# fperezgamonal/flownet2-tf

Measured on AMD Instinct MI355X. Metric: forward pairs/sec at 512x384 (FlowNet2), higher is better.
Workload: dtype f16x2 (split fp16 hi+lo operands, 3 fp16 MFMAs per product, fp32 accumulate); 1 GPU; FlowNet2 forward, batch=4 synthetic 512x384 pairs per GPU, seeded synthetic weights; pairs_per_gpu=4, parallelism=dp1 (no collective)

## Files before the change

### flownet2-tf_amd/csrc/conv.hip

```cpp
#include "conv_common.h"
#include <cstdlib>

namespace fn2 {

template <typename T, typename OutT, int TC, int WC, int WP>
__global__ void __launch_bounds__(256) conv_igemm_kernel(const ConvArgs p) {
  constexpr int CH = 16 / (int)sizeof(T);
  constexpr int BC = WC * TC * 16;
  constexpr int BP = WP * 64;
  constexpr int NT = 256;
  static_assert(WC * WP == 4, "4 waves per block");
  constexpr int NPR = BP / 64;
  constexpr int NWR = (BC * 4 + NT - 1) / NT;
  constexpr int WSWZ_BIT = (TC == 4) ? 5 : (TC == 2) ? 4 : 3;
  __shared__ uint4 lds[2][(BC + BP) * 4];

  const int tid = threadIdx.x, lane = tid & 63, wave = tid >> 6;
  const int wc = wave / WP, wp = wave % WP;
  const int cid = tid & 3;

  int pad_y = p.pad, pad_x = p.pad, oy_off = 0, ox_off = 0, osc = 1;
  const T* wgt = reinterpret_cast<const T*>(p.wgt);
  const int phase = blockIdx.z / p.splitk, split = blockIdx.z - phase * p.splitk;
  if (p.deconv) {
// ... 970 lines not shown
  {
    const double A = (double)d->cout_pad * d->kpad * esz, B = (double)d->in.n * d->in.h * d->in.w * d->in.cs * esz;
    const long X = cdiv(M, 64), Y = cdiv(d->cout_pad, 128);
    const char* e = getenv("FN2_WMAJOR");
    const int mode = e ? atoi(e) : 2;
    a.wmajor = mode == 2 ? (A * (double)(X < 8 ? X : 8) + B > A + B * (double)(Y < 8 ? Y : 8)) : mode;
  }
  a.bp64 = wfrag ? 1 : wants_bp64(a, tile, phases, d->wgt_layout) ? 1 : 0;
  if ((a.dbg & 64) && d->wgt_layout == 1 && tile == 128 && !a.bp64) a.bp64 = 2;
  if (wfrag) {
    const char* e_wr = getenv("FN2_WREG_RING");
    const char* e_ring = getenv("FN2_RING_MAX");
    const int mode = e_wr ? atoi(e_wr) : 1;
    const long blocks = (long)cdiv(a.M, 64) * (a.cout_pad / 128) * phases;
    if (tile == 128 && (mode == 2 || (mode == 1 && blocks >= 384 && blocks <= (e_ring ? atoi(e_ring) : 512)))) a.wfrag = 2;
  }
  a.kg = 1;
  if (d->wgt_layout == 1 && tile == 128 && !(a.dbg & 32)) {
    const char* e_kg = getenv("FN2_KG");
    if (!e_kg || atoi(e_kg) != 0) {
      const char* e3 = getenv("FN2_KG3_MAX");
      const char* e2 = getenv("FN2_KG2_MAX");
      const long blocks = (long)cdiv(a.M, 64) * (a.cout_pad / 128) * phases;
      if (blocks <= (e3 ? atoi(e3) : 0)) { a.bp64 = 1; a.kg = 3; }
      else if (blocks <= (e2 ? atoi(e2) : 95)) { a.bp64 = 1; a.kg = 2; }
    }
  }
  if (d->wgt_layout == 1 && tile == 128 && !(a.dbg & 32) && d->in.dtype == FN2_F16X2) {
    const char* e_lo = getenv("FN2_DEEP_MIN");
    const char* e_hi = getenv("FN2_DEEP_MAX");
// ... 2 lines not shown
    if (blocks >= lo && blocks <= hi) { a.bp64 = 3; a.kg = 1; }
  }
  if (d->wgt_layout == 1 && tile == 128 && a.bp64 == 1 && a.kg == 1) {
    const char* e_ring = getenv("FN2_RING_MAX");
    const int ring_max = e_ring ? atoi(e_ring) : 512;
    const long blocks = (long)cdiv(a.M, 64) * (a.cout_pad / 128) * phases;
    if ((a.dbg & 256) || (blocks >= 384 && blocks <= ring_max)) a.bp64 = 2;
    const char* e_rs = getenv("FN2_RING_SPLIT");
    if (e_rs && blocks >= atoi(e_rs) && blocks < 384) a.bp64 = 2;
  }
  *tile_out = tile;
  *phases_out = phases;
  return FN2_OK;
}

static int preferred_split(const ConvArgs& a, int tile, int phases) {
  if (a.merged) return 1;
  const int bp = tile == 128 ? (a.bp64 ? 64 : 128) : (a.bp64 ? 128 : 256);
  const long blocks = (long)cdiv(a.M, bp) * (a.cout_pad / tile) * phases;
  const char* e_min = getenv("FN2_SPLIT_MINBLOCKS");
  if (blocks >= (e_min ? atoi(e_min) : 384)) return 1;
  if (a.bp64 == 3) {
    const char* e_sl = getenv("FN2_DEEP_SLOTS");
    int s = (int)((e_sl ? atoi(e_sl) : 256) / blocks);
    const int maxs = a.ksteps / 16;
    if (s > maxs) s = maxs;
    if (s > 16) s = 16;
    if (s < 2) return 1;
    const int kper = cdiv(a.ksteps, s);
    return cdiv(a.ksteps, kper);
  }
  if (a.kg > 1) {
// ... 101 lines not shown
  if (d->up_src != nullptr && d->kind == 5 && 2 * d->out.c == 32) {
    a.up_src = d->up_src; a.up_w = d->up_w; a.up_bias = d->up_bias; a.up_c0 = d->up_c0;
  }
  if (d->head != nullptr && !conv_name_sink().buf) {
    const fn2_conv_desc* h = reinterpret_cast<const fn2_conv_desc*>(d->head);
    FN2_REQUIRE(d->kind == 1 && is_flow_head(h) && h->head == nullptr && h->up_src == nullptr,
                "conv2d: head rides on a kind-1 transposed conv and is a 3x3 two-output fp32 flow head");
    FN2_REQUIRE(h->in.data == d->in.data && h->in.n == d->in.n && h->in.h == d->in.h && h->in.w == d->in.w &&
                    h->in.cs == d->in.cs && h->in.c0 == d->in.c0 && h->in.dtype == d->in.dtype,
                "conv2d: head and transposed conv must read the same view");
    ConvArgs ha;
    int htile, hphases;
    rc = build_args(h, &ha, &htile, &hphases);
    if (rc) return rc;
    const char* e = getenv("FN2_HEAD_RIDE");
    const bool ride = d->in.dtype == FN2_F16X2 && d->wgt_layout == 2 && tile == 128 && sk > 1 && !(e && atoi(e) == 0);
    if (ride) {
      a.fh_M = ha.M;
      a.fh_w = reinterpret_cast<const float*>(ha.wgt);
      a.fh_w1 = ha.ksteps * 4 * 4;
      a.fh_groups = ha.cin_chunks >> 1;
      a.fh_bias = ha.bias;
      a.fh_out = reinterpret_cast<float*>(ha.out);
      a.fh_out_cs = ha.out_cs; a.fh_out_c0 = ha.out_c0;
      a.fh_scale = ha.out_scale;
    } else {
      rc = fn2_conv2d(h, stream);
      if (rc) return rc;
    }
  }
  if (d->wgt_layout >= 1) {
// ... 220 lines not shown
```

### flownet2-tf_amd/csrc/conv2.hip

```cpp
#include "conv_common.h"

#include <type_traits>
#include <algorithm>
#include <utility>

#ifndef FN2_X2_ORDER
#define FN2_X2_ORDER 0
#endif
#ifndef FN2_CONV_ABLATE
#define FN2_CONV_ABLATE 0
#endif
#ifndef FN2_SETPRIO
#define FN2_SETPRIO 1
#endif

namespace fn2 {

typedef __attribute__((address_space(3))) void* lptr_t;

constexpr unsigned kOobOffset = 0x80000000u;

typedef int v4i_t __attribute__((ext_vector_type(4)));
typedef unsigned u32x4_t __attribute__((ext_vector_type(4)));

// ... 74 lines not shown
  for (int k = 0; k < 4; ++k) {
    const long m = (long)rb * 16 + wave * 4 + k;
    if (m >= total) return;
    h5_ring_pixel(p, m);
  }
}

__device__ __forceinline__ float* h5_t(uint4* a, uint4* b, int half, int w) {
  const int byte = w * 4;
  return byte < half ? reinterpret_cast<float*>(reinterpret_cast<char*>(a) + byte)
                     : reinterpret_cast<float*>(reinterpret_cast<char*>(b) + (byte - half));
}

template <typename T, typename OutT, int WC, int WP, int TCN = 2, int TPN = 2, int STAGES = 2, int KG = 1, bool M16 = false,
          bool WREG = false, bool SLAB = false, bool HEAD5 = false, bool FEED = false>
__global__ void __launch_bounds__(256 * KG + (FEED ? 256 : 0)) conv_igemm2_kernel(const ConvArgs p) {
#if defined(__HIP_DEVICE_COMPILE__)
  constexpr int CH = 16 / (int)sizeof(T);
  constexpr int ESZ = (int)sizeof(T);
  constexpr int BC = WC * TCN * 32, BP = WP * TPN * 32;
  static_assert(WC * WP == 4, "4 waves per block");
  constexpr int NWI = BC / 32;
  constexpr int NPI = BP / 32;
  static_assert(!WREG || (is_x2<T>::value && TCN == 1 && KG == 1 && (STAGES == 2 || STAGES == 3) && !M16),
                "WREG: split fp16, one cout tile per wave, two-stage loop or 3-slot ring");
  constexpr int BOFF = WREG ? 0 : BC;
  constexpr int kWTileBytes = (32 * TPN * (TCN * 32 + 4) + 32 * TPN) * 4;
  constexpr int kPoolHalfRows = (STAGES * BP * 128 / 2 > 2 * kWTileBytes ? STAGES * BP * 128 / 2 : 2 * kWTileBytes) / 128 + 1;
  constexpr int ROWS = WREG ? kPoolHalfRows : BC + BP;
  static_assert(KG == 1 || STAGES == 2, "K groups run the two-stage loop");
  constexpr bool kDeep = STAGES > 3;
  __shared__ uint4 lds0_all[(kDeep ? STAGES : WREG ? 2 : KG) * ROWS * 8];
  __shared__ uint4 lds1_all[(kDeep || WREG) ? 1 : KG * ROWS * 8];
  __shared__ uint4 lds2_own[(STAGES == 3 && !WREG) ? ROWS * 8 : 1];

  if constexpr (HEAD5) {
    if ((int)blockIdx.x >= p.h5_tiles) {
      h5_ring_block(p, (int)blockIdx.x - p.h5_tiles);
      return;
    }
  }
  if constexpr (WREG && SLAB && is_x2<T>::value) {
    if (p.fh_M > 0 && (int)blockIdx.z >= p.fh_z0) {
      if (FEED && threadIdx.x >= 256) return;
      float* part = reinterpret_cast<float*>(lds0_all);
      const long e = (((long)blockIdx.z - p.fh_z0) * gridDim.y + blockIdx.y) * gridDim.x + blockIdx.x;
      const long total = (long)(gridDim.z - p.fh_z0) * gridDim.y * gridDim.x;
      for (long m = e; m < p.fh_M; m += total)
        fh_pixel(reinterpret_cast<const x2_t*>(p.in), p.H, p.W, p.in_cs, p.in_c0, p.fh_groups, p.fh_w, p.fh_w + p.fh_w1,
                 p.fh_bias, p.fh_scale, p.fh_out + (size_t)m * p.fh_out_cs + p.fh_out_c0, m, part);
      return;
    }
  }
  const int tid = threadIdx.x, lane = tid & 63;
  const int wave_all = __builtin_amdgcn_readfirstlane(tid >> 6);
  const int grp = KG > 1 ? wave_all >> 2 : 0;
  static_assert(!FEED || (WREG && STAGES == 3 && KG == 1), "FEED: the WREG ring");
  const bool feeder = FEED && wave_all >= 4;
  const int wave = (KG > 1 || FEED) ? wave_all & 3 : wave_all;
  uint4* const lds0 = lds0_all + grp * (ROWS * 8);
  uint4* const lds1 = WREG ? lds0_all + BP * 8 : kDeep ? lds0_all + ROWS * 8 : lds1_all + grp * (ROWS * 8);
  uint4* const lds2 = WREG ? lds0_all + 2 * BP * 8 : lds2_own;
  uint4* const ep1 = (kDeep || WREG) ? lds0_all + ROWS * 8 : lds1_all;
  const int wc = wave / WP, wp = wave % WP;

  int pad_y = p.pad, pad_x = p.pad, oy_off = 0, ox_off = 0, osc = 1;
  const T* wgt = reinterpret_cast<const T*>(p.wgt);
  const int phase = blockIdx.z / p.splitk, split = blockIdx.z - phase * p.splitk;
  const unsigned wrow_bytes = (unsigned)p.ksteps * 128u;
  if (p.deconv) {
    const int a = phase >> 1, b = phase & 1;
    pad_y = a ? p.ph_pad1 : p.ph_pad0; pad_x = b ? p.ph_pad1 : p.ph_pad0; oy_off = a; ox_off = b; osc = 2;
    wgt += (size_t)phase * p.cout_pad * (wrow_bytes / ESZ);
  }
  const int khi = p.deconv ? p.kh_ph[phase >> 1] : p.KH, kwi = p.deconv ? p.kw_ph[phase & 1] : p.KW;
  const int nst_all = (p.cin_chunks >> 3) * khi * kwi;
// ... 17 lines not shown

  const v4i_t rsrc_w = make_rsrc(wgt, (int)(p.cout_pad * wrow_bytes));
  const v4i_t rsrc_x = make_rsrc(p.in, p.in_bytes);

  const int lrow = lane >> 3, lphys = lane & 7;
  unsigned woff[NWI];
#pragma unroll
  for (int j = 0; j < NWI; ++j) {
    const int row = wave * (BC / 4) + j * 8 + lrow;
    woff[j] = (unsigned)(c0 + row) * wrow_bytes + (unsigned)((lphys ^ ((row >> 1) & 7)) * 16);
  }
  int roff[NPI];
  unsigned vmask[NPI];
#pragma unroll
  for (int j = 0; j < NPI; ++j) {
    const int row = wave * (BP / 4) + j * 8 + lrow;
    const int m = m0 + row;
    bool v = m < p.M;
    const int mm = v ? m : 0;
    int n = mm / (p.OH * p.OW);
    const int rem = mm - n * (p.OH * p.OW);
    int oy = rem / p.OW, ox = rem - oy * p.OW;
    if constexpr (HEAD5) {
      static_assert(BP == 256, "HEAD5: 8 x 32 positions per block");
      const int tx = bx % p.h5_tx, tyn = bx / p.h5_tx;
      n = tyn / p.h5_ty;
      oy = (tyn - n * p.h5_ty) * 4 - 2 + (row >> 5);
      ox = tx * 28 - 2 + (row & 31);
      v = true;
    }
    const int iy0 = oy * p.stride - pad_y, ix0 = ox * p.stride - pad_x;
// ... 14 lines not shown
  int wstage = kt0;

  auto issue_piece = [&](auto piece_c, uint4* lds) {
    constexpr int i = decltype(piece_c)::value;
    if constexpr (i < NWI) {
      if constexpr (!WREG) {
        if (!(FN2_CONV_ABLATE && (p.dbg & 2)))
          dma16(rsrc_w, &lds[(wave * (BC / 4) + i * 8) * 8], woff[i], ((ky * p.KW + kx) * spt + sc) * 128);
      }
    } else {
      constexpr int j = i - NWI;
      const unsigned tbit = (1u << ky) | (1u << (8 + kx));
      const int toff = ((ky * p.W + kx) * p.in_cs + sc * 8 * CH) * ESZ;
      const unsigned voff = ((vmask[j] & tbit) == tbit && wstage < kt1) ? (unsigned)(roff[j] + toff) : kOobOffset;
      if (!(FN2_CONV_ABLATE && (p.dbg & 1)))
        dma16(rsrc_x, &lds[(BOFF + wave * (BP / 4) + j * 8) * 8], voff, 0);
    }
  };
  u32x4_t wfa[WREG ? 4 : 1], wfb[WREG ? 4 : 1], wfc[(WREG && STAGES == 3) ? 4 : 1];
  const unsigned wlane = (unsigned)lane * 16u;
  const int wtile_off = WREG ? ((c0 >> 5) + wc) * (p.ksteps * 4096) : 0;
  auto load_w = [&](u32x4_t (&wf)[WREG ? 4 : 1]) {
    if constexpr (WREG) {
      const int soff = wtile_off + ((ky * p.KW + kx) * spt + sc) * 4096;
      asm volatile("buffer_load_dwordx4 %0, %4, %5, %6 offen\n\t"
                   "buffer_load_dwordx4 %1, %4, %5, %6 offen offset:1024\n\t"
                   "buffer_load_dwordx4 %2, %4, %5, %6 offen offset:2048\n\t"
                   "buffer_load_dwordx4 %3, %4, %5, %6 offen offset:3072"
                   : "=&v"(wf[0]), "=&v"(wf[1]), "=&v"(wf[2]), "=&v"(wf[3])
                   : "v"(wlane), "s"(rsrc_w), "s"(soff) : "memory");
    }
// ... 206 lines not shown
    };
    issue_stage_w(lds0, wfa);
    issue_stage_w(lds1, wfb);
    const int nst3 = (kt1 - kt0 + 2) / 3 * 3;
    for (int s = 0; s < nst3; s += 3) {
      ring_sync_w(wfa); issue_stage_w(lds2, wfc); compute_w(lds0, wfa);
      ring_sync_w(wfb); issue_stage_w(lds0, wfa); compute_w(lds1, wfb);
      ring_sync_w(wfc); issue_stage_w(lds1, wfb); compute_w(lds2, wfc);
    }
    asm volatile("s_waitcnt vmcnt(0)" : "+v"(wfa[0]), "+v"(wfa[1]), "+v"(wfa[2]), "+v"(wfa[3]), "+v"(wfb[0]), "+v"(wfb[1]),
                 "+v"(wfb[2]), "+v"(wfb[3]) :: "memory");
  } else if constexpr (WREG) {
    issue_stage_w(lds0, wfa);
    wait_w(wfa);
    __syncthreads();
    const int nst2 = (kt1 - kt0 + 1) & ~1;
    for (int s = 0; s < nst2; s += 2) {
      issue_stage_w(lds1, wfb);
      compute_w(lds0, wfa);
      wait_w(wfb);
      __syncthreads();
      if (s + 2 < nst2) issue_stage_w(lds0, wfa);
      compute_w(lds1, wfb);
      wait_w(wfa);
      __syncthreads();
    }
  } else if constexpr (STAGES == 2) {
    issue_stage(lds0);
    asm volatile("s_waitcnt vmcnt(0)" ::: "memory");
    __syncthreads();
    const int nst2 = ((kt1 - (kt0 - grp) + KG - 1) / KG + 1) & ~1;
// ... 32 lines not shown
      else asm volatile("s_waitcnt vmcnt(8)\n\ts_barrier" ::: "memory");
    };
    issue_stage(lds0);
    issue_stage(lds1);
    const int nst3 = (kt1 - kt0 + 2) / 3 * 3;
    for (int s = 0; s < nst3; s += 3) {
      ring_sync(); issue_stage(lds2); compute(lds0);
      ring_sync(); issue_stage(lds0); compute(lds1);
      ring_sync(); issue_stage(lds1); compute(lds2);
    }
    asm volatile("s_waitcnt vmcnt(0)" ::: "memory");
  }

  if constexpr (KG > 1) {
    constexpr int NA4 = TCN * TPN * 4;
    static_assert((KG - 1) * 4 * NA4 * 64 <= KG * ROWS * 8, "reduction scratch must fit the stage buffers");
    float4* red = reinterpret_cast<float4*>(lds0_all);
    auto acc4 = [&](int idx) -> float4 {
      if constexpr (M16) {
        const f32x4 v = acc16[idx / (TPN * 2)][idx % (TPN * 2)];
        return make_float4(v[0], v[1], v[2], v[3]);
      } else {
        const int t = idx >> 2, q = idx & 3;
        return make_float4(acc[t / TPN][t % TPN][4 * q], acc[t / TPN][t % TPN][4 * q + 1], acc[t / TPN][t % TPN][4 * q + 2],
                           acc[t / TPN][t % TPN][4 * q + 3]);
      }
    };
    if (grp > 0) {
#pragma unroll
      for (int idx = 0; idx < NA4; ++idx) red[(((grp - 1) * 4 + wave) * NA4 + idx) * 64 + lane] = acc4(idx);
    }
    __syncthreads();
    if (grp > 0) return;
#pragma unroll
    for (int g = 0; g < KG - 1; ++g)
#pragma unroll
      for (int idx = 0; idx < NA4; ++idx) {
        const float4 v = red[((g * 4 + wave) * NA4 + idx) * 64 + lane];
        if constexpr (M16) {
          f32x4& d = acc16[idx / (TPN * 2)][idx % (TPN * 2)];
          d[0] += v.x; d[1] += v.y; d[2] += v.z; d[3] += v.w;
        } else {
          const int t = idx >> 2, q = idx & 3;
          acc[t / TPN][t % TPN][4 * q] += v.x; acc[t / TPN][t % TPN][4 * q + 1] += v.y;
          acc[t / TPN][t % TPN][4 * q + 2] += v.z; acc[t / TPN][t % TPN][4 * q + 3] += v.w;
        }
      }
  }

  if constexpr (HEAD5) {
    if (p.dbg & 2) return;
    constexpr int TS = 52;
    static_assert(256 * TS * 4 <= 2 * ROWS * 128, "T fits the stage buffers");
// ... 66 lines not shown
          v[j] = x;
        }
        if (p.vec_ok && co + 3 < p.Cout) store_vec<OutT, 4>(po + co, v);
        else
#pragma unroll
          for (int j = 0; j < 4; ++j)
            if (co + j < p.Cout) store_elem<OutT>(po + co + j, v[j]);
      }
    }
    return;
  }

  OutT* out = reinterpret_cast<OutT*>(p.out);
  constexpr int WCOLS = TCN * 32, RS = WCOLS + 4, WROWS = 32 * TPN;
  constexpr int WTW = WROWS * RS + WROWS;
  constexpr bool kLdsT = (KG > 1 ? 4 : 2) * WTW * 4 <= KG * ROWS * 128;
  if constexpr (FEED && !kLdsT) { if (feeder) return; }
  float* const tl = reinterpret_cast<float*>(KG > 1 ? ep1 : (wave < 2 ? lds0_all : ep1)) + (KG > 1 ? wave : (wave & 1)) * WTW;
  constexpr int CPR = WCOLS / 4, RPI = 64 / CPR;
  static_assert(!SLAB || WREG, "SLAB is a specialisation of the WREG instantiations");
  if ((SLAB || !WREG) && p.splitk > 1) {
    float* slab = p.ws + (size_t)split * p.N * p.out_H * p.out_W * p.ws_cs;
    if constexpr (kLdsT) {
      if constexpr (STAGES >= 3) __syncthreads();
      if constexpr (FEED) { if (feeder) return; }
      int* rowoff = reinterpret_cast<int*>(tl + WROWS * RS);
#pragma unroll
      for (int tp = 0; tp < TPN; ++tp) {
        const int m = m0 + wp * TPN * 32 + tp * 32 + fr;
        const int mm = m < p.M ? m : 0;
        const int n = mm / (p.OH * p.OW);
        const int rem = mm - n * (p.OH * p.OW);
        const int oy = rem / p.OW, ox = rem - oy * p.OW;
// ... 810 lines not shown
  const char* e_m16 = getenv("FN2_M16_MIN");
  const bool m16 = is_x2<T>::value && !(a.dbg & 512) &&
                   ((a.dbg & 1024) || (e_m16 && tile == 128 && a.bp64 == 1 && a.kg == 1 && a.splitk == 1 &&
                                       blocks64 >= atoi(e_m16)));
#define FN2_LAUNCH2(GX, GY, THREADS, ...)                                                              \
  do {                                                                                                 \
    dim3 grid(GX, GY, z);                                                                              \
    if (conv_name_sink().buf)                                                                          \
      snprintf(conv_name_sink().buf, conv_name_sink().cap, "conv_igemm2_kernel<%s, %s, %s, %s>", type_name<T>(), \
               type_name<OutT>(), #__VA_ARGS__, m16 ? "true" : "false");                              \
    else if (m16) hipLaunchKernelGGL((conv_igemm2_kernel<T, OutT, __VA_ARGS__, is_x2<T>::value>), grid, dim3(THREADS), 0, s, a); \
    else hipLaunchKernelGGL((conv_igemm2_kernel<T, OutT, __VA_ARGS__, false>), grid, dim3(THREADS), 0, s, a);            \
  } while (0)
  if (a.wfrag) {
    if constexpr (is_x2<T>::value) {
      if (tile == 64) {
        dim3 grid(cdiv(a.M, 128), a.cout_pad / 64, z);
        if (conv_name_sink().buf)
          snprintf(conv_name_sink().buf, conv_name_sink().cap, "conv_igemm2_kernel<%s, %s, 2, 2, 1, 2, 2, 1, false, true, %s>",
                   type_name<T>(), type_name<OutT>(), a.splitk > 1 ? "true" : "false");
        else if (a.splitk > 1)
          hipLaunchKernelGGL((conv_igemm2_kernel<T, OutT, 2, 2, 1, 2, 2, 1, false, true, true>), grid, dim3(256), 0, s, a);
        else
          hipLaunchKernelGGL((conv_igemm2_kernel<T, OutT, 2, 2, 1, 2, 2, 1, false, true, false>), grid, dim3(256), 0, s, a);
      } else {
        dim3 grid(cdiv(a.M, 64), a.cout_pad / 128, z);
        const bool slab = a.splitk > 1;
        ConvArgs ah = a;
        if (a.fh_M > 0 && slab && !conv_name_sink().buf) {
          const char* e = getenv("FN2_FH_BLOCKS");
          const long per_z = (long)grid.x * grid.y;
          const long want = std::min<long>(a.fh_M, e ? atoi(e) : 1024);
          ah.fh_z0 = z;
          grid.z = z + (unsigned)std::max<long>(1, (want + per_z - 1) / per_z);
        } else {
          ah.fh_M = 0;
        }
        const ConvArgs& a = ah;
        const char* e_feed = getenv("FN2_WREG_FEED");
        const int feed = e_feed ? atoi(e_feed) : 1;
        if (conv_name_sink().buf)
          snprintf(conv_name_sink().buf, conv_name_sink().cap, "conv_igemm2_kernel<%s, %s, 4, 1, 1, 2, %d, 1, false, true, %s%s>",
                   type_name<T>(), type_name<OutT>(), a.wfrag == 2 ? 3 : 2, slab ? "true" : "false",
                   (a.wfrag == 2 && (slab ? feed >= 2 : feed >= 1)) ? ", false, true" : "");
        else if (a.wfrag == 2 && slab && feed >= 2)
          hipLaunchKernelGGL((conv_igemm2_kernel<T, OutT, 4, 1, 1, 2, 3, 1, false, true, true, false, true>), grid, dim3(512), 0, s, a);
        else if (a.wfrag == 2 && slab)
          hipLaunchKernelGGL((conv_igemm2_kernel<T, OutT, 4, 1, 1, 2, 3, 1, false, true, true>), grid, dim3(256), 0, s, a);
        else if (a.wfrag == 2 && feed >= 1)
          hipLaunchKernelGGL((conv_igemm2_kernel<T, OutT, 4, 1, 1, 2, 3, 1, false, true, false, false, true>), grid, dim3(512), 0, s, a);
        else if (a.wfrag == 2)
          hipLaunchKernelGGL((conv_igemm2_kernel<T, OutT, 4, 1, 1, 2, 3, 1, false, true, false>), grid, dim3(256), 0, s, a);
        else if (slab)
          hipLaunchKernelGGL((conv_igemm2_kernel<T, OutT, 4, 1, 1, 2, 2, 1, false, true, true>), grid, dim3(256), 0, s, a);
        else
          hipLaunchKernelGGL((conv_igemm2_kernel<T, OutT, 4, 1, 1, 2, 2, 1, false, true, false>), grid, dim3(256), 0, s, a);
// ... 64 lines not shown
```

### flownet2-tf_amd/csrc/conv_common.h

```cpp
#pragma once
#include "fn2_common.h"

namespace fn2 {

struct ConvArgs {
  const void* in;
  const void* wgt;
  const float* bias;
  void* out;
  int N, H, W, in_cs, in_c0;
  int cin_chunks;
  int KH, KW, stride, pad;
  int OH, OW;
  int M;
  int out_H, out_W, out_cs, out_c0, Cout;
  int ksteps;
  int cout_pad;
  int act;
  int deconv;
  int ph_pad0, ph_pad1;
  int kh_ph[2], kw_ph[2];
  int merged;
  int wmajor;
  int bp64;
// ... 1 lines not shown
  int kg;
  int h5_tx, h5_ty, h5_ring;
  int h5_tiles, h5_groups;
  const float* h5_wc;
  const float* h5_bc;
  int h5_rows;
  int fh_M, fh_z0;
  const float* fh_w;
  int fh_w1, fh_groups;
  const float* fh_bias;
  float* fh_out;
  int fh_out_cs, fh_out_c0;
  float fh_scale;
  const float* up_src; const float* up_w; const float* up_bias; int up_c0;
  int wfrag;
  int accum;
  int vec_ok;
  int splitk;
  int kper;
  float* ws;
  int ws_cs;
  float out_scale;
  int in_bytes;
  const void* mask_y;
  int mask_c0, mask_c1;
  int dbg;
};

__device__ __forceinline__ void fh_pixel(const x2_t* __restrict__ in, int H, int W, int in_cs, int in_c0, int groups,
                                         const float* __restrict__ wf0, const float* __restrict__ wf1,
// ... 93 lines not shown
```

### flownet2-tf_amd/src/_hip.py

```python
import ctypes as C
import os

import numpy as np
import torch

_HERE = os.path.dirname(os.path.abspath(__file__))
LIB_PATH = os.path.join(os.path.dirname(_HERE), "lib", "libflownet2_hip.so")

FN2_F32, FN2_BF16, FN2_F16, FN2_F16X2 = 0, 1, 2, 3
ACT_NONE, ACT_LEAKY = 0, 1
OK = 0
ERR_INVALID_ARGUMENT, ERR_UNSUPPORTED, ERR_HIP = -1, -2, -3


class Fn2Tensor(C.Structure):
    _fields_ = [("data", C.c_void_p), ("dtype", C.c_int32), ("n", C.c_int32), ("h", C.c_int32),
                ("w", C.c_int32), ("c", C.c_int32), ("cs", C.c_int32), ("c0", C.c_int32)]


class Fn2ConvPlan(C.Structure):
    _fields_ = [("layout", C.c_int32), ("cout_tile", C.c_int32), ("kstep_elems", C.c_int32),
                ("wgt_dtype", C.c_int32)]


class Fn2ConvDesc(C.Structure):
    _fields_ = [("inp", Fn2Tensor), ("out", Fn2Tensor), ("wgt", C.c_void_p), ("bias", C.c_void_p),
                ("kind", C.c_int32), ("kh", C.c_int32), ("kw", C.c_int32), ("stride", C.c_int32),
                ("pad", C.c_int32), ("act", C.c_int32), ("cin_pad", C.c_int32), ("cout_pad", C.c_int32),
                ("kpad", C.c_int32), ("wgt_layout", C.c_int32), ("accumulate", C.c_int32), ("out_scale", C.c_float), ("workspace", C.c_void_p), ("workspace_bytes", C.c_int64),
                ("act_grad_y", C.c_void_p), ("act_grad_c0", C.c_int32), ("act_grad_c1", C.c_int32),
                ("up_src", C.c_void_p), ("up_w", C.c_void_p), ("up_bias", C.c_void_p), ("up_c0", C.c_int32),
                ("head", C.c_void_p), ("raw_partials", C.c_int32)]


class Fn2BwdwDesc(C.Structure):
    _fields_ = [("x", Fn2Tensor), ("dy", Fn2Tensor), ("dw", C.c_void_p), ("kind", C.c_int32), ("kh", C.c_int32),
                ("kw", C.c_int32), ("stride", C.c_int32), ("pad", C.c_int32), ("cin_pad", C.c_int32),
                ("cout_pad", C.c_int32), ("kpad", C.c_int32), ("wgt_layout", C.c_int32), ("db", C.c_void_p)]


_i, _p, _f = C.c_int, C.c_void_p, C.c_float
_ip = C.POINTER(C.c_int)
_tp = C.POINTER(Fn2Tensor)

PROTOTYPES = {
    "fn2_last_error": (C.c_char_p, []),
    "fn2_version": (_i, []),
# ... 150 lines not shown
```

### flownet2-tf_amd/src/engine.py

```python
import ctypes as C
import math
import os

import numpy as np
import torch

from . import _hip, netdefs, weights as W

_DT = {"f32": torch.float32, "bf16": torch.bfloat16, "f16": torch.float16, "f16x2": torch.float32}
_CODE = {"f32": _hip.FN2_F32, "bf16": _hip.FN2_BF16, "f16": _hip.FN2_F16, "f16x2": _hip.FN2_F16X2}
_TILE_ARGS = {128: "2, 2, 2, 2", 64: "1, 4, 2, 2", 32: "1, 4, 1, 2"}


def conv2_kernel_args(tile, m, cout_pad, phases, x2=True):
    dbg = int(os.environ.get("FN2_CONV_DBG", "0"))
    blocks64 = -(-m // 64) * (cout_pad // 128) * phases if tile == 128 else 0
    big = "FN2_M16_MIN" in os.environ and blocks64 >= max(int(os.environ["FN2_M16_MIN"]), 513)
    m16 = "true" if (x2 and not dbg & 512 and (dbg & 1024 or big)) else "false"
    full = dbg & 32
    if tile < 128:
        base = {64: "1, 4, 2, 2, 2, 1", 32: "1, 4, 1, 2, 2, 1"}[tile] if full else {64: "1, 4, 2, 1, 2, 1", 32: "1, 4, 1, 1, 2, 1"}[tile]
        return f"{base}, {m16}"
    blocks = -(-m // 64) * (cout_pad // 128) * phases
    if not full and int(os.environ.get("FN2_KG", "1")):
# ... 15 lines not shown


class BatchTooLarge(ValueError):

    def __init__(self, name, batch, nbytes, limit):
        self.fit = max(1, int(batch * (limit - 1) // nbytes))
        super().__init__("activation tensor %s of a batch of %d pairs is %d bytes (limit %d): at most %d pairs per engine"
                         % (name, batch, nbytes, limit, self.fit))


class Engine:
    MAX_TENSOR_BYTES = 1 << 31

    def __init__(self, model, weights, batch, height, width, dtype="f32", device=None, heads_as_gemm=True,
                 no_deconv_biases=None, strict=True, uint8_inputs=False, plain_stems=False, fragment_weights=None,
                 interp_u8_inputs=False):
        if model not in netdefs.MODELS:
            raise ValueError("unknown model %r" % model)
        if dtype not in _DT:
            raise ValueError("dtype must be 'f32', 'bf16', 'f16' or 'f16x2'")
        if height % 64 or width % 64:
            raise ValueError("height and width must be multiples of 64 (pad with Net.adapt_x, net.py:373-388)")
        self.lib = _hip.lib()
        self.device = device if device is not None else _hip.require_device()
        self.model, self.N, self.H, self.W = model, int(batch), int(height), int(width)
        self.dtype_name, self.tdtype = dtype, _DT[dtype]
        self.act_code = _CODE[dtype]
        self.code_of = {}
        self.weights = weights
        if no_deconv_biases is None:
            no_deconv_biases = "FlowNetS/predict_flow6/biases" not in weights
# ... 33 lines not shown
        self.interp_u8_inputs = bool(interp_u8_inputs)
        if self.interp_u8_inputs:
            if model != "FlowNetS_interp":
                raise ValueError("interp_u8_inputs belongs to FlowNetS_interp, not %s" % model)
            self.in_img_u8 = torch.zeros((self.N, self.H, self.W, 3), dtype=torch.uint8, device=self.device)
            self.in_mask_u8 = torch.zeros((self.N, self.H, self.W), dtype=torch.uint8, device=self.device)
            self.in_sparse = torch.zeros((self.N, self.H, self.W, 2), dtype=torch.float32, device=self.device)
            self.in_flags = torch.ones((self.N, 2), dtype=torch.uint8, device=self.device)
            self._lut_255 = torch.from_numpy((np.arange(256, dtype=np.float64) / 255.0).astype(np.float32)).to(self.device)
        self.graph = None
        self.conv_descs = []
        self.layers = []
        self.heads_as_gemm = heads_as_gemm
        self.plain_stems = bool(plain_stems)
        self.fragment_weights = bool(int(os.environ.get("FN2_WREG", "1"))) if fragment_weights is None else bool(fragment_weights)
        self.compose_heads = bool(heads_as_gemm) and dtype == "f16x2" and bool(int(os.environ.get("FN2_COMPOSE", "1")))
        self._head_t = None
        self._defer_flow = False
        self._own_ws = set()
        self._pending_head = None
        self.outputs = self._build()
        assert self._pending_head is None
        self._check_variables(strict)
        self._alloc_workspace()
        self._resolve_kernel_names()

    def _buf(self, name, n, h, w, c, dtype=None, stem=False):
        line = 64 if self.act_code in (_hip.FN2_BF16, _hip.FN2_F16) else 32
        cs = (_round_up(c, line) if c > 32 else _round_up(c, 8)) if dtype is None else c
        if dtype is None and not stem and line == 32 and 8 < c <= 32:
# ... 114 lines not shown
                packed = packed * (2.0 ** k2)
                out_scale = 2.0 ** (-k2)
        wdev = W.packed_to_device(packed, plan.wgt_dtype, self.device)
        d = _hip.Fn2ConvDesc()
        d.inp = self._v(sbuf, sc, sc0)
        d.out = self._v(dbuf, dc, dc0)
        d.wgt = wdev.data_ptr()
        d.bias = bias.data_ptr() if bias is not None else None
        d.kind = 0 if kind == "conv" else (5 if merged else 1)
        d.kh = d.kw = k
        d.stride, d.pad = stride, pad
        d.act = _hip.ACT_LEAKY if act else _hip.ACT_NONE
        d.cin_pad, d.cout_pad, d.kpad = cin_pad, cout_pad, kpad
        d.wgt_layout = layout
        d.out_scale = out_scale
        frag = False
        if (self.fragment_weights and layout == 1 and tile >= int(os.environ.get("FN2_WREG_TILE_MIN", "128"))
                and plan.wgt_dtype == _hip.FN2_F16X2 and self._wants_fragments(d)):
            wdev = W.to_fragment_order(wdev)
            d.wgt, d.wgt_layout, frag = wdev.data_ptr(), 2, True
        self.keep += [d, wdev, bias]
        self.conv_descs.append(d)
        self.desc_branch.append(self._branch)
        up_rec = None
        if self._pending_head is not None and kind != "conv":
            hd = self._pending_head
            assert up_after is not None and hd.inp.data == d.inp.data and hd.inp.c0 == d.inp.c0, (scope, name)
            d.head = C.addressof(hd)
            self._pending_head = None
        if up_after is not None:
# ... 775 lines not shown
```

### flownet2-tf_amd/src/trainer.py

```python
import ctypes as C
import math
import os

import numpy as np
import torch

from . import _hip, weights as W
from .engine import Engine, _round_up
from .training_schedules import LONG_SCHEDULE

LOSS_WEIGHTS = {6: 0.32, 5: 0.08, 4: 0.02, 3: 0.01, 2: 0.005}
F32 = _hip.FN2_F32


def _index_hwio(rec):
    if "_hwio_index" in rec:
        return rec["_hwio_index"]
    rec["_hwio_index"] = _index_hwio_uncached(rec)
    return rec["_hwio_index"]


def _index_hwio_uncached(rec):
    kind = rec["kind"]
    if kind == 1:
# ... 31 lines not shown
        if model == "FlowNetC" and dtype != "f32":
            raise ValueError("FlowNetC trains in dtype 'f32' (the correlation gradient op is fp32)")
        self.model = model
        self.train_scope = scopes[model]
        self.hfem = (add_hard_flow_mining or "").lower()
        if self.hfem not in ("", "hard", "edges"):
            raise ValueError("add_hard_flow_mining must be '', 'hard' or 'edges'")
        self.lambda_w, self.hard_perc = float(lambda_weight), float(hard_examples_perc)
        self.gt_scale = 20.0 if model == "FlowNetSD" else 0.05
        self.loss_terms = {"predict_flow%d" % lvl: wgt / 5.0 for lvl, wgt in LOSS_WEIGHTS.items()}
        if model == "FlowNet2":
            self.loss_terms, self.gt_scale = {"predict_flow0": 1.0}, 1.0
            if self.hfem:
                raise ValueError("hard-flow-example mining belongs to FlowNetS_interp")
        self.eng = Engine(model, weights, batch, height, width, dtype, heads_as_gemm=False, plain_stems=True,
                          fragment_weights=self.x2 and bool(int(os.environ.get("FN2_TRAIN_WREG", "0"))))
        self.lib, self.dev = self.eng.lib, self.eng.device
        self.N, self.H, self.W = batch, height, width
        self.schedule, self.eps = schedule, eps
        self.step_count = 0
        self.keep = []
        self.gt = torch.zeros((batch, height, width, 2), dtype=torch.float32, device=self.dev)
        self.loss_dev = torch.zeros(1, dtype=torch.float32, device=self.dev)
        self._build()

    def _gbuf(self, buf):
        key = buf.untyped_storage().data_ptr()
        if key not in self.gbufs:
            base = self.base_of[key]
            self.gbufs[key] = torch.zeros_like(base)
        g = self.gbufs[key]
# ... 252 lines not shown
                                                      dtype=np.float64)
        gmap = torch.from_numpy((pk.reshape(-1) - 1.0).astype(np.int32)).to(self.dev)
        wb = torch.zeros(gmap.numel(), dtype=torch.float32, device=self.dev)
        scale = rec.get("scale", 1.0)
        gather = [wb, rec["master"], gmap, scale, 0]
        self.gathers.append(gather)
        d = _hip.Fn2ConvDesc()
        d.inp = self._view(gy_buf, gy_c, gy_c0)
        d.out = self._view(gx_buf, gx_c, gx_c0)
        d.wgt, d.bias = wb.data_ptr(), None
        d.kind, d.kh, d.kw, d.stride, d.pad = kind, k, k, stride, pad
        d.act = _hip.ACT_NONE
        d.cin_pad, d.cout_pad, d.kpad, d.wgt_layout = cin_pad, cout_pad, kpad, plan.layout
        d.accumulate = 1
        d.out_scale = 1.0 / scale
        if self.eng.fragment_weights and plan.layout == 1 and plan.cout_tile == 128 and self.eng._wants_fragments(d):
            d.wgt_layout, gather[4] = 2, kpad
        self.keep += [d, wb, gmap]
        self.eng.conv_descs.append(d)
        tn = "fn2::x2_t" if self.x2 else "float"
        if plan.layout == 1:
            from .engine import conv2_kernel_args
            gxs = gx_buf.shape
            m_px = gxs[0] * gxs[1] * gxs[2] // (4 if kind == 3 else 1)
            d.kernel_name = "conv_igemm2_kernel<%s, %s, %s>" % (tn, tn, conv2_kernel_args(plan.cout_tile, m_px, cout_pad,
                                                                                               4 if kind == 3 else 1, self.x2))
        else:
            d.kernel_name = "conv_igemm_kernel<float, float, %s>" % {128: "4, 2, 2", 64: "4, 1, 4", 32: "2, 1, 4",
                                                                      16: "1, 1, 4"}[plan.cout_tile]
        return d
# ... 430 lines not shown
```

### include/flownet2_hip.h

```cpp
#ifndef FLOWNET2_HIP_H_
#define FLOWNET2_HIP_H_

#include <stddef.h>
#include <stdint.h>

#ifdef __cplusplus
extern "C" {
#endif

typedef enum {
  FN2_OK = 0,
  FN2_ERR_INVALID_ARGUMENT = -1,
  FN2_ERR_UNSUPPORTED = -2,
  FN2_ERR_HIP = -3
} fn2_status;

typedef enum { FN2_F32 = 0, FN2_BF16 = 1, FN2_F16 = 2, FN2_F16X2 = 3 } fn2_dtype;

typedef enum { FN2_ACT_NONE = 0, FN2_ACT_LEAKY = 1  } fn2_act;

typedef struct {
  void* data;
  int32_t dtype;
  int32_t n, h, w;
// ... 53 lines not shown
  int32_t cout_pad;
  int32_t kpad;
  int32_t wgt_layout;
  int32_t accumulate;
  float out_scale;
  void* workspace;
  int64_t workspace_bytes;
  const void* act_grad_y;
  int32_t act_grad_c0, act_grad_c1;
  const float* up_src;
  const float* up_w;
  const float* up_bias;
  int32_t up_c0;
  const void* head;
  int32_t raw_partials;
} fn2_conv_desc;

typedef struct {
  int32_t layout, cout_tile, kstep_elems, wgt_dtype;
} fn2_conv_plan;
int fn2_conv2d_plan(int in_dtype, int cin_pad, int cout, fn2_conv_plan* plan);
int64_t fn2_conv2d_workspace_bytes(const fn2_conv_desc* d);
int fn2_conv2d(const fn2_conv_desc* d, void* stream);
int fn2_conv2d_kernel_name(const fn2_conv_desc* desc, char* name, int cap);
int fn2_conv2d_splits(const fn2_conv_desc* desc);

int fn2_flow_head_gather(const float* t, int t_cs, const float* bias, float* out, int n, int h, int w, void* stream);
int fn2_flow_head_tail(const float* t, int t_cs, int taps, const float* bias, float* pf, int n, int h, int w, int ring,
                       const float* up_w, const float* up_bias, const fn2_tensor* up_out, void* stream);
int fn2_flow_head_tail_slabs(const float* t, int t_cs, int nslab, int64_t slab_stride, float scale, int taps, const float* bias,
// ... 86 lines not shown
```

Baseline: 1118 pairs/s.

## Add K-pair WREG conv variant splitting K across wave pairs for small grids

```diff
diff --git a/flownet2-tf_amd/csrc/conv.hip b/flownet2-tf_amd/csrc/conv.hip
--- a/flownet2-tf_amd/csrc/conv.hip
+++ b/flownet2-tf_amd/csrc/conv.hip
@@ -1008,6 +1008,14 @@
     const int mode = e_wr ? atoi(e_wr) : 1;
     const long blocks = (long)cdiv(a.M, 64) * (a.cout_pad / 128) * phases;
     if (tile == 128 && (mode == 2 || (mode == 1 && blocks >= 384 && blocks <= (e_ring ? atoi(e_ring) : 512)))) a.wfrag = 2;
+    const char* e_kp = getenv("FN2_KPAIR");
+    const char* e_kpmax = getenv("FN2_KPAIR_MAX");
+    const char* e_kpmin = getenv("FN2_KPAIR_MIN");
+    const char* e_kptile = getenv("FN2_KPAIR_TILE_MIN");
+    const long blocks128 = (long)cdiv(a.M, 64) * cdiv(a.cout_pad, 128) * phases;
+    if (tile >= (e_kptile ? atoi(e_kptile) : 128) && a.wfrag == 1 && !d->no_k_pair && !(e_kp && atoi(e_kp) == 0) &&
+        blocks128 >= (e_kpmin ? atoi(e_kpmin) : 0) && blocks128 <= (e_kpmax ? atoi(e_kpmax) : 95))
+      a.kpair = 1;
   }
   a.kg = 1;
   if (d->wgt_layout == 1 && tile == 128 && !(a.dbg & 32)) {
@@ -1040,8 +1048,24 @@
   return FN2_OK;
 }
 
-static int preferred_split(const ConvArgs& a, int tile, int phases) {
+static int preferred_split(ConvArgs& a, int tile, int phases) {
   if (a.merged) return 1;
+  if (a.kpair) {
+    const char* e_sl = getenv("FN2_SPLIT_SLOTS");
+    const char* e_ms = getenv("FN2_KPAIR_MINSTAGES");
+    const char* e_min = getenv("FN2_SPLIT_MINBLOCKS");
+    const long blocks = (long)cdiv(a.M, 64) * cdiv(a.cout_pad, 128) * phases;
+    const int ms = e_ms && atoi(e_ms) > 0 ? atoi(e_ms) : 4;
+    int s = blocks >= (e_min ? atoi(e_min) : 384) ? 1 : (int)((e_sl ? atoi(e_sl) : 640) / blocks);
+    if (s > 16) s = 16;
+    s /= 2;
+    if (s > a.ksteps / (4 * ms)) s = a.ksteps / (4 * ms);
+    if (s >= 2) {
+      const int kper = cdiv(a.ksteps, s);
+      return cdiv(a.ksteps, kper);
+    }
+    a.kpair = 0;
+  }
   const int bp = tile == 128 ? (a.bp64 ? 64 : 128) : (a.bp64 ? 128 : 256);
   const long blocks = (long)cdiv(a.M, bp) * (a.cout_pad / tile) * phases;
   const char* e_min = getenv("FN2_SPLIT_MINBLOCKS");
@@ -1173,7 +1197,7 @@
     rc = build_args(h, &ha, &htile, &hphases);
     if (rc) return rc;
     const char* e = getenv("FN2_HEAD_RIDE");
-    const bool ride = d->in.dtype == FN2_F16X2 && d->wgt_layout == 2 && tile == 128 && sk > 1 && !(e && atoi(e) == 0);
+    const bool ride = d->in.dtype == FN2_F16X2 && d->wgt_layout == 2 && (tile == 128 || a.kpair) && sk > 1 && !(e && atoi(e) == 0);
     if (ride) {
       a.fh_M = ha.M;
       a.fh_w = reinterpret_cast<const float*>(ha.wgt);
diff --git a/flownet2-tf_amd/csrc/conv2.hip b/flownet2-tf_amd/csrc/conv2.hip
--- a/flownet2-tf_amd/csrc/conv2.hip
+++ b/flownet2-tf_amd/csrc/conv2.hip
@@ -112,19 +112,22 @@
 
 template <typename T, typename OutT, int WC, int WP, int TCN = 2, int TPN = 2, int STAGES = 2, int KG = 1, bool M16 = false,
           bool WREG = false, bool SLAB = false, bool HEAD5 = false, bool FEED = false>
-__global__ void __launch_bounds__(256 * KG + (FEED ? 256 : 0)) conv_igemm2_kernel(const ConvArgs p) {
+__global__ void __launch_bounds__(256 * (WREG ? 1 : KG) + (FEED ? 256 : 0)) conv_igemm2_kernel(const ConvArgs p) {
 #if defined(__HIP_DEVICE_COMPILE__)
   constexpr int CH = 16 / (int)sizeof(T);
   constexpr int ESZ = (int)sizeof(T);
   constexpr int BC = WC * TCN * 32, BP = WP * TPN * 32;
-  static_assert(WC * WP == 4, "4 waves per block");
+  constexpr bool KPAIR = WREG && KG == 2;
+  constexpr int GW = KPAIR ? 2 : 4;
+  static_assert(WC * WP == GW, "4 waves per block (K pair: two per K half)");
   constexpr int NWI = BC / 32;
-  constexpr int NPI = BP / 32;
-  static_assert(!WREG || (is_x2<T>::value && TCN == 1 && KG == 1 && (STAGES == 2 || STAGES == 3) && !M16),
+  constexpr int NPI = BP / (8 * GW);
+  static_assert(!WREG || (is_x2<T>::value && TCN == 1 && (KG == 1 || KG == 2) && (STAGES == 2 || STAGES == 3) && !M16),
                 "WREG: split fp16, one cout tile per wave, two-stage loop or 3-slot ring");
+  static_assert(!KPAIR || (SLAB && STAGES == 2 && WP == 1 && !FEED), "K pair: the split-K form of the two-stage loop");
   constexpr int BOFF = WREG ? 0 : BC;
   constexpr int kWTileBytes = (32 * TPN * (TCN * 32 + 4) + 32 * TPN) * 4;
-  constexpr int kPoolHalfRows = (STAGES * BP * 128 / 2 > 2 * kWTileBytes ? STAGES * BP * 128 / 2 : 2 * kWTileBytes) / 128 + 1;
+  constexpr int kPoolHalfRows = (KG * STAGES * BP * 128 / 2 > 2 * kWTileBytes ? KG * STAGES * BP * 128 / 2 : 2 * kWTileBytes) / 128 + 1;
   constexpr int ROWS = WREG ? kPoolHalfRows : BC + BP;
   static_assert(KG == 1 || STAGES == 2, "K groups run the two-stage loop");
   constexpr bool kDeep = STAGES > 3;
@@ -152,12 +155,12 @@
   }
   const int tid = threadIdx.x, lane = tid & 63;
   const int wave_all = __builtin_amdgcn_readfirstlane(tid >> 6);
-  const int grp = KG > 1 ? wave_all >> 2 : 0;
+  const int grp = KPAIR ? wave_all >> 1 : KG > 1 ? wave_all >> 2 : 0;
   static_assert(!FEED || (WREG && STAGES == 3 && KG == 1), "FEED: the WREG ring");
   const bool feeder = FEED && wave_all >= 4;
-  const int wave = (KG > 1 || FEED) ? wave_all & 3 : wave_all;
-  uint4* const lds0 = lds0_all + grp * (ROWS * 8);
-  uint4* const lds1 = WREG ? lds0_all + BP * 8 : kDeep ? lds0_all + ROWS * 8 : lds1_all + grp * (ROWS * 8);
+  const int wave = KPAIR ? wave_all & 1 : (KG > 1 || FEED) ? wave_all & 3 : wave_all;
+  uint4* const lds0 = lds0_all + grp * (WREG ? 2 * BP * 8 : ROWS * 8);
+  uint4* const lds1 = WREG ? lds0 + BP * 8 : kDeep ? lds0_all + ROWS * 8 : lds1_all + grp * (ROWS * 8);
   uint4* const lds2 = WREG ? lds0_all + 2 * BP * 8 : lds2_own;
   uint4* const ep1 = (kDeep || WREG) ? lds0_all + ROWS * 8 : lds1_all;
   const int wc = wave / WP, wp = wave % WP;
@@ -205,7 +208,7 @@
   unsigned vmask[NPI];
 #pragma unroll
   for (int j = 0; j < NPI; ++j) {
-    const int row = wave * (BP / 4) + j * 8 + lrow;
+    const int row = wave * (BP / GW) + j * 8 + lrow;
     const int m = m0 + row;
     bool v = m < p.M;
     const int mm = v ? m : 0;
@@ -250,7 +253,7 @@
       const int toff = ((ky * p.W + kx) * p.in_cs + sc * 8 * CH) * ESZ;
       const unsigned voff = ((vmask[j] & tbit) == tbit && wstage < kt1) ? (unsigned)(roff[j] + toff) : kOobOffset;
       if (!(FN2_CONV_ABLATE && (p.dbg & 1)))
-        dma16(rsrc_x, &lds[(BOFF + wave * (BP / 4) + j * 8) * 8], voff, 0);
+        dma16(rsrc_x, &lds[(BOFF + wave * (BP / GW) + j * 8) * 8], voff, 0);
     }
   };
   u32x4_t wfa[WREG ? 4 : 1], wfb[WREG ? 4 : 1], wfc[(WREG && STAGES == 3) ? 4 : 1];
@@ -487,7 +490,7 @@
     issue_stage_w(lds0, wfa);
     wait_w(wfa);
     __syncthreads();
-    const int nst2 = (kt1 - kt0 + 1) & ~1;
+    const int nst2 = ((kt1 - (kt0 - grp) + KG - 1) / KG + 1) & ~1;
     for (int s = 0; s < nst2; s += 2) {
       issue_stage_w(lds1, wfb);
       compute_w(lds0, wfa);
@@ -550,8 +553,8 @@
 
   if constexpr (KG > 1) {
     constexpr int NA4 = TCN * TPN * 4;
-    static_assert((KG - 1) * 4 * NA4 * 64 <= KG * ROWS * 8, "reduction scratch must fit the stage buffers");
-    float4* red = reinterpret_cast<float4*>(lds0_all);
+    static_assert((KG - 1) * GW * NA4 * 64 <= (KPAIR ? 1 : KG) * ROWS * 8, "reduction scratch must fit the stage buffers");
+    float4* red = reinterpret_cast<float4*>(KPAIR ? ep1 : lds0_all);
     auto acc4 = [&](int idx) -> float4 {
       if constexpr (M16) {
         const f32x4 v = acc16[idx / (TPN * 2)][idx % (TPN * 2)];
@@ -564,7 +567,7 @@
     };
     if (grp > 0) {
 #pragma unroll
-      for (int idx = 0; idx < NA4; ++idx) red[(((grp - 1) * 4 + wave) * NA4 + idx) * 64 + lane] = acc4(idx);
+      for (int idx = 0; idx < NA4; ++idx) red[(((grp - 1) * GW + wave) * NA4 + idx) * 64 + lane] = acc4(idx);
     }
     __syncthreads();
     if (grp > 0) return;
@@ -572,7 +575,7 @@
     for (int g = 0; g < KG - 1; ++g)
 #pragma unroll
       for (int idx = 0; idx < NA4; ++idx) {
-        const float4 v = red[((g * 4 + wave) * NA4 + idx) * 64 + lane];
+        const float4 v = red[((g * GW + wave) * NA4 + idx) * 64 + lane];
         if constexpr (M16) {
           f32x4& d = acc16[idx / (TPN * 2)][idx % (TPN * 2)];
           d[0] += v.x; d[1] += v.y; d[2] += v.z; d[3] += v.w;
@@ -669,9 +672,9 @@
   OutT* out = reinterpret_cast<OutT*>(p.out);
   constexpr int WCOLS = TCN * 32, RS = WCOLS + 4, WROWS = 32 * TPN;
   constexpr int WTW = WROWS * RS + WROWS;
-  constexpr bool kLdsT = (KG > 1 ? 4 : 2) * WTW * 4 <= KG * ROWS * 128;
+  constexpr bool kLdsT = KPAIR ? 2 * WTW * 4 <= ROWS * 128 : (KG > 1 ? 4 : 2) * WTW * 4 <= KG * ROWS * 128;
   if constexpr (FEED && !kLdsT) { if (feeder) return; }
-  float* const tl = reinterpret_cast<float*>(KG > 1 ? ep1 : (wave < 2 ? lds0_all : ep1)) + (KG > 1 ? wave : (wave & 1)) * WTW;
+  float* const tl = reinterpret_cast<float*>((KG > 1 && !KPAIR) ? ep1 : (wave < 2 ? lds0_all : ep1)) + ((KG > 1 && !KPAIR) ? wave : (wave & 1)) * WTW;
   constexpr int CPR = WCOLS / 4, RPI = 64 / CPR;
   static_assert(!SLAB || WREG, "SLAB is a specialisation of the WREG instantiations");
   if ((SLAB || !WREG) && p.splitk > 1) {
@@ -1512,7 +1515,8 @@
   } while (0)
   if (a.wfrag) {
     if constexpr (is_x2<T>::value) {
-      if (tile == 64) {
+      const bool kpair = a.kpair && a.splitk > 1 && a.wfrag == 1;
+      if (tile == 64 && !kpair) {
         dim3 grid(cdiv(a.M, 128), a.cout_pad / 64, z);
         if (conv_name_sink().buf)
           snprintf(conv_name_sink().buf, conv_name_sink().cap, "conv_igemm2_kernel<%s, %s, 2, 2, 1, 2, 2, 1, false, true, %s>",
@@ -1522,8 +1526,8 @@
         else
           hipLaunchKernelGGL((conv_igemm2_kernel<T, OutT, 2, 2, 1, 2, 2, 1, false, true, false>), grid, dim3(256), 0, s, a);
       } else {
-        dim3 grid(cdiv(a.M, 64), a.cout_pad / 128, z);
         const bool slab = a.splitk > 1;
+        dim3 grid(cdiv(a.M, 64), a.cout_pad / (kpair ? 64 : 128), z);
         ConvArgs ah = a;
         if (a.fh_M > 0 && slab && !conv_name_sink().buf) {
           const char* e = getenv("FN2_FH_BLOCKS");
@@ -1537,7 +1541,12 @@
         const ConvArgs& a = ah;
         const char* e_feed = getenv("FN2_WREG_FEED");
         const int feed = e_feed ? atoi(e_feed) : 1;
-        if (conv_name_sink().buf)
+        if (conv_name_sink().buf && kpair)
+          snprintf(conv_name_sink().buf, conv_name_sink().cap, "conv_igemm2_kernel<%s, %s, 2, 1, 1, 2, 2, 2, false, true, true>",
+                   type_name<T>(), type_name<OutT>());
+        else if (kpair)
+          hipLaunchKernelGGL((conv_igemm2_kernel<T, OutT, 2, 1, 1, 2, 2, 2, false, true, true>), grid, dim3(256), 0, s, a);
+        else if (conv_name_sink().buf)
           snprintf(conv_name_sink().buf, conv_name_sink().cap, "conv_igemm2_kernel<%s, %s, 4, 1, 1, 2, %d, 1, false, true, %s%s>",
                    type_name<T>(), type_name<OutT>(), a.wfrag == 2 ? 3 : 2, slab ? "true" : "false",
                    (a.wfrag == 2 && (slab ? feed >= 2 : feed >= 1)) ? ", false, true" : "");
diff --git a/flownet2-tf_amd/csrc/conv_common.h b/flownet2-tf_amd/csrc/conv_common.h
--- a/flownet2-tf_amd/csrc/conv_common.h
+++ b/flownet2-tf_amd/csrc/conv_common.h
@@ -39,6 +39,7 @@
   float fh_scale;
   const float* up_src; const float* up_w; const float* up_bias; int up_c0;
   int wfrag;
+  int kpair;
   int accum;
   int vec_ok;
   int splitk;
diff --git a/flownet2-tf_amd/src/_hip.py b/flownet2-tf_amd/src/_hip.py
--- a/flownet2-tf_amd/src/_hip.py
+++ b/flownet2-tf_amd/src/_hip.py
@@ -30,7 +30,7 @@
                 ("kpad", C.c_int32), ("wgt_layout", C.c_int32), ("accumulate", C.c_int32), ("out_scale", C.c_float), ("workspace", C.c_void_p), ("workspace_bytes", C.c_int64),
                 ("act_grad_y", C.c_void_p), ("act_grad_c0", C.c_int32), ("act_grad_c1", C.c_int32),
                 ("up_src", C.c_void_p), ("up_w", C.c_void_p), ("up_bias", C.c_void_p), ("up_c0", C.c_int32),
-                ("head", C.c_void_p), ("raw_partials", C.c_int32)]
+                ("head", C.c_void_p), ("raw_partials", C.c_int32), ("no_k_pair", C.c_int32)]
 
 
 class Fn2BwdwDesc(C.Structure):
diff --git a/flownet2-tf_amd/src/engine.py b/flownet2-tf_amd/src/engine.py
--- a/flownet2-tf_amd/src/engine.py
+++ b/flownet2-tf_amd/src/engine.py
@@ -53,7 +53,7 @@
 
     def __init__(self, model, weights, batch, height, width, dtype="f32", device=None, heads_as_gemm=True,
                  no_deconv_biases=None, strict=True, uint8_inputs=False, plain_stems=False, fragment_weights=None,
-                 interp_u8_inputs=False):
+                 interp_u8_inputs=False, k_pair=True):
         if model not in netdefs.MODELS:
             raise ValueError("unknown model %r" % model)
         if dtype not in _DT:
@@ -117,6 +117,7 @@
         self.heads_as_gemm = heads_as_gemm
         self.plain_stems = bool(plain_stems)
         self.fragment_weights = bool(int(os.environ.get("FN2_WREG", "1"))) if fragment_weights is None else bool(fragment_weights)
+        self.k_pair = bool(k_pair)
         self.compose_heads = bool(heads_as_gemm) and dtype == "f16x2" and bool(int(os.environ.get("FN2_COMPOSE", "1")))
         self._head_t = None
         self._defer_flow = False
@@ -261,6 +262,7 @@
         d.cin_pad, d.cout_pad, d.kpad = cin_pad, cout_pad, kpad
         d.wgt_layout = layout
         d.out_scale = out_scale
+        d.no_k_pair = 0 if self.k_pair else 1
         frag = False
         if (self.fragment_weights and layout == 1 and tile >= int(os.environ.get("FN2_WREG_TILE_MIN", "128"))
                 and plan.wgt_dtype == _hip.FN2_F16X2 and self._wants_fragments(d)):
diff --git a/flownet2-tf_amd/src/trainer.py b/flownet2-tf_amd/src/trainer.py
--- a/flownet2-tf_amd/src/trainer.py
+++ b/flownet2-tf_amd/src/trainer.py
@@ -69,7 +69,7 @@
             if self.hfem:
                 raise ValueError("hard-flow-example mining belongs to FlowNetS_interp")
         self.eng = Engine(model, weights, batch, height, width, dtype, heads_as_gemm=False, plain_stems=True,
-                          fragment_weights=self.x2 and bool(int(os.environ.get("FN2_TRAIN_WREG", "0"))))
+                          fragment_weights=self.x2 and bool(int(os.environ.get("FN2_TRAIN_WREG", "0"))), k_pair=False)
         self.lib, self.dev = self.eng.lib, self.eng.device
         self.N, self.H, self.W = batch, height, width
         self.schedule, self.eps = schedule, eps
@@ -352,6 +352,7 @@
         d.cin_pad, d.cout_pad, d.kpad, d.wgt_layout = cin_pad, cout_pad, kpad, plan.layout
         d.accumulate = 1
         d.out_scale = 1.0 / scale
+        d.no_k_pair = 1
         if self.eng.fragment_weights and plan.layout == 1 and plan.cout_tile == 128 and self.eng._wants_fragments(d):
             d.wgt_layout, gather[4] = 2, kpad
         self.keep += [d, wb, gmap]
diff --git a/include/flownet2_hip.h b/include/flownet2_hip.h
--- a/include/flownet2_hip.h
+++ b/include/flownet2_hip.h
@@ -91,6 +91,7 @@
   int32_t up_c0;
   const void* head;
   int32_t raw_partials;
+  int32_t no_k_pair;
 } fn2_conv_desc;
 
 typedef struct {
```

Measured after the change: 1127 pairs/s, median of 6. About the same (+0.8%).
